# olivier-2018/scene_3Dreconstruction_MVSNet

Hardware: AMD Instinct MI355X
Metric: depth maps/sec at N=5 views, 640x512, D=192; achieved HBM GB/s (higher is better)
Workload: dtype f32 (conv0, conv2-4, conv9, conv11: 3xbf16 split operands on the bf16 matrix cores, fp32 accumulate)

## Files before the change

scene_3dreconstruction_mvsnet_amd/csrc/conv11_prob.hip:

```cpp
#include <cstdlib>

#include "mvs_internal.h"
#include "storage.h"
#include "mfma16_ops.h"

namespace mvs {

namespace cp {
constexpr int BY = 4, BX = 2;
constexpr int IY = 2 * BY, IX = 8 * BX;
constexpr int OY = 2 * IY, OX = 2 * IX;
constexpr int PY = OY - 2, PX = OX - 2;

constexpr int XP = 36;
constexpr int HS = XP * 4, RS = 2 * HS, PS = (OY + 2) * RS;
constexpr int C_FLOATS = 2 * PS;

constexpr int WSLOTS = 69;
__host__ __device__ constexpr int win_slot(int rho, int c) {
    return c < 8 ? 8 * rho + c : rho == 0 ? 52 : rho == 1 ? 48 : rho == 2 ? 56 : rho == 3 ? 60 : rho == 4 ? 68 : 64;
}
}

namespace cpv {
using namespace cp;
constexpr int RPI = 76;
constexpr int WIN = 2 * 3 * RPI;
constexpr int NPC = 2 * 27 * 2;
}

template <int DT>
__global__ __launch_bounds__(512, 4) void conv11_prob_priv_kernel(
    const void* __restrict__ x, const float* __restrict__ bp, const float* __restrict__ bias,
    const void* __restrict__ skip, const float* __restrict__ pw, const float* __restrict__ pbias,
    float* __restrict__ cost, int Di, int Hi, int Wi, int ZC, int nbx, int nby) {
    using namespace cpv;
    __shared__ __attribute__((aligned(16))) float ct[C_FLOATS];
    __shared__ __attribute__((aligned(16))) float win[8 * WIN];
    __shared__ __attribute__((aligned(16))) float bpan[2 * 9 * 64 * 4];

    const int tid = threadIdx.x, lane = tid & 63, wave = tid >> 6;
    int b = xcd_block();
    const int bx = b % nbx; b /= nbx;
    const int by = b % nby;
    const int bz = b / nby;
    const int ix0 = bx * (IX - 1), iy0 = by * (IY - 1);
    const int za = bz * ZC, zb = min(za + ZC, Di);
    const int Do = 2 * Di, Ho = 2 * Hi, Wo = 2 * Wi;
    const size_t Vin = (size_t)Di * Hi * Wi, HWi = (size_t)Hi * Wi, HWo = (size_t)Ho * Wo;
    const int i_first = za > 0 ? za - 1 : 0, i_last = zb < Di ? zb : Di - 1;

    const int tx = wave & 1, ty = wave >> 1;
    float* my = win + wave * WIN;
    int prel[2], ploff[2];
    unsigned pin = 0, phz = 0;
#pragma unroll
    for (int j = 0; j < 2; ++j) {
        const int p = lane + 64 * j;
        const int half = p & 1, v = p >> 1, hz = v / 27, vv = v % 27, hr = vv / 9, hc = vv % 9;
        const int gy = iy0 + 2 * ty + hr, gx = ix0 + 8 * tx + hc;
        const bool ok = p < NPC && gy < Hi && gx < Wi;
        prel[j] = ok ? (int)((((size_t)hz * Hi + gy) * Wi + gx) * 8 + half * 4) : 0;
        pin |= ok ? (1u << j) : 0u;
        phz |= (hz & 1) ? (1u << j) : 0u;
        ploff[j] = p < NPC ? (hz * 3 + hr) * RPI + hc * 8 + half * 4 : -1;
    }
    f32x4 pre[2];
    bool pre_z1 = true;
    auto load_a = [&](int i, int c) {
        pre_z1 = i + 1 < Di;
        const size_t base = ((size_t)c * Vin + (size_t)i * HWi) * 8;
#pragma unroll
        for (int j = 0; j < 2; ++j) {
            const bool ok = ((pin >> j) & 1u) && (pre_z1 || !((phz >> j) & 1u));
            pre[j] = St<DT>::load4(x, ok ? base + prel[j] : (size_t)0);
        }
    };
    auto store_a = [&]() {
#pragma unroll
        for (int j = 0; j < 2; ++j) {
            const bool ok = ((pin >> j) & 1u) && (pre_z1 || !((phz >> j) & 1u));
            if (ploff[j] >= 0) *reinterpret_cast<f32x4*>(my + ploff[j]) = ok ? pre[j] : (f32x4){0.f, 0.f, 0.f, 0.f};
        }
    };
    const int r = lane & 15, g = lane >> 4;
    const int abase = (r >> 3) * RPI + ((r & 7) + (g >> 1)) * 8 + (g & 1) * 4;
    const int px = r >> 3, co = r & 7;
    const float bv = bias[co];
    const int sbase0 = (2 * (2 * ty + (g >> 1)) + 1) * RS + (co >> 2) * HS + (2 * (8 * tx + 4 * (g & 1)) + px + 1) * 4 + (co & 3);
    int srel[4], sl[4];
    unsigned sok = 0;
#pragma unroll
    for (int j = 0; j < 4; ++j) {
        const int xx = lane & 15, half = (lane >> 4) & 1, rr = 2 * (j & 1) + (lane >> 5), pz = j >> 1;
        const int oy = 4 * ty + rr, ox = 16 * tx + xx;
        const int gy = 2 * iy0 + oy, gx = 2 * ix0 + ox;
        const bool ok = gy < Ho && gx < Wo;
        srel[j] = ok ? (int)((((size_t)pz * Ho + gy) * Wo + gx) * 8 + half * 4) : 0;
        sok |= ok ? (1u << j) : 0u;
        sl[j] = pz * PS + (oy + 1) * RS + half * HS + (ox + 1) * 4;
    }
    f32x4 sk[4];
    auto load_skip = [&](int i, bool de, bool dodd) {
        const size_t base = (size_t)(2 * i) * HWo * 8;
#pragma unroll
        for (int j = 0; j < 4; ++j) {
            const bool ok = ((sok >> j) & 1u) && ((j >> 1) ? dodd : de);
            sk[j] = St<DT>::load4(skip, ok ? base + srel[j] : (size_t)0);
        }
    };
    const f32x4* bsrc = reinterpret_cast<const f32x4*>(bpan) + lane;
    f32x4 acc[4];
    auto fetch = [&](int c, int ks, f32x4& a, f32x4& bq) {
        const DeconvStep st = deconv_step(ks);
        a = *reinterpret_cast<const f32x4*>(my + (st.dz * 3 + st.dy) * RPI + abase);
        bq = bsrc[(c * 9 + ks) * 64];
    };
    auto mfma_step = [&](int ks, const f32x4& a, const f32x4& bq) {
        const int cls = deconv_step(ks).cls;
        acc[cls] = __builtin_amdgcn_mfma_f32_16x16x4f32(a.x, bq.x, acc[cls], 0, 0, 0);
        acc[cls] = __builtin_amdgcn_mfma_f32_16x16x4f32(a.y, bq.y, acc[cls], 0, 0, 0);
        acc[cls] = __builtin_amdgcn_mfma_f32_16x16x4f32(a.z, bq.z, acc[cls], 0, 0, 0);
        acc[cls] = __builtin_amdgcn_mfma_f32_16x16x4f32(a.w, bq.w, acc[cls], 0, 0, 0);
    };
    auto mfma_chunk = [&](int c, bool de, bool dodd) {
        if (de && dodd) {
            f32x4 a[2], bq[2];
            fetch(c, 0, a[0], bq[0]);
#pragma unroll
            for (int ks = 0; ks < 9; ++ks) {
                if (ks + 1 < 9) fetch(c, ks + 1, a[(ks + 1) & 1], bq[(ks + 1) & 1]);
                mfma_step(ks, a[ks & 1], bq[ks & 1]);
            }
        } else {
#pragma unroll
            for (int ks = 0; ks < 9; ++ks) {
                if (deconv_step(ks).cls < 2 ? !de : !dodd) continue;
                f32x4 a, bq;
                fetch(c, ks, a, bq);
                mfma_step(ks, a, bq);
            }
        }
    };

    const int lx = tid & 31, ly = tid >> 5;
    const int gyo = 2 * iy0 + ly, gxo = 2 * ix0 + lx;
    const bool pvalid = gyo < Ho && gxo < Wo && (ly >= 1 || iy0 == 0) && (ly <= OY - 2 || gyo == Ho - 1) &&
                        (lx >= 1 || ix0 == 0) && (lx <= OX - 2 || gxo == Wo - 1);
    const size_t pout = (size_t)gyo * Wo + gxo;
    const int cbase = ly * RS + lx * 4;
    auto stencil = [&](int plane, f32x2& k2, f32x2& k1, f32x2& k0) {
        const float* base = ct + plane * PS + cbase;
#pragma unroll 1
        for (int kx = 0; kx < 3; ++kx) {
            f32x4 v[3][2];
#pragma unroll
            for (int rr = 0; rr < 3; ++rr)
#pragma unroll
                for (int hf = 0; hf < 2; ++hf)
                    v[rr][hf] = *reinterpret_cast<const f32x4*>(base + rr * RS + hf * HS + kx * 4);
#pragma unroll
            for (int ky = 0; ky < 3; ++ky) {
                const float* w2 = pw + ((2 * 3 + ky) * 3 + kx) * 8;
                const float* w1 = pw + ((1 * 3 + ky) * 3 + kx) * 8;
                const float* w0 = pw + ((0 * 3 + ky) * 3 + kx) * 8;
#pragma unroll
                for (int c2 = 0; c2 < 4; ++c2) {
                    const f32x4 q = v[ky][c2 >> 1];
                    const f32x2 d = (c2 & 1) ? (f32x2){q.z, q.w} : (f32x2){q.x, q.y};
                    k2 = __builtin_elementwise_fma(d, (f32x2){w2[2 * c2], w2[2 * c2 + 1]}, k2);
                    k1 = __builtin_elementwise_fma(d, (f32x2){w1[2 * c2], w1[2 * c2 + 1]}, k1);
                    k0 = __builtin_elementwise_fma(d, (f32x2){w0[2 * c2], w0[2 * c2 + 1]}, k0);
                }
            }
        }
    };
    const __amdgpu_buffer_rsrc_t crs = __builtin_amdgcn_make_buffer_rsrc(cost, (short)0, (int)((size_t)Do * HWo * 4), 0x00020000);
    auto emit = [&](int oz, const f32x2& sv, bool live) {
        const unsigned off = (pvalid && live) ? (unsigned)(((size_t)oz * HWo + pout) * 4) : 0xFFFFFFFCu;
        __builtin_amdgcn_raw_buffer_store_b32(__builtin_bit_cast(unsigned, sv.x + sv.y), crs, (int)off, 0, 0);
    };

    const float pb = pbias[0];
    const f32x2 fresh = {pb, 0.0f};
    f32x2 A = fresh, B = fresh, C = fresh;

    for (int k = tid; k < C_FLOATS / 4; k += 512) reinterpret_cast<f32x4*>(ct)[k] = (f32x4){0.f, 0.f, 0.f, 0.f};
    for (int k = tid; k < 2 * 9 * 64; k += 512) reinterpret_cast<f32x4*>(bpan)[k] = reinterpret_cast<const f32x4*>(bp)[k];
    load_a(i_first, 0);
    __builtin_amdgcn_sched_barrier(0);
    load_skip(i_first, i_first >= za, i_first < zb);
    __syncthreads();

#pragma unroll 1
    for (int i = i_first; i <= i_last; ++i) {
        const bool de = i >= za, dodd = i < zb;
        store_a();
        __builtin_amdgcn_wave_barrier();
        __builtin_amdgcn_sched_barrier(0);
        load_a(i, 1);
        __builtin_amdgcn_sched_barrier(0);
#pragma unroll
        for (int c = 0; c < 4; ++c) acc[c] = (f32x4){0.f, 0.f, 0.f, 0.f};
        mfma_chunk(0, de, dodd);
        __builtin_amdgcn_wave_barrier();
        __builtin_amdgcn_sched_barrier(0);
        store_a();
        __builtin_amdgcn_wave_barrier();
        __builtin_amdgcn_sched_barrier(0);
        load_a(min(i + 1, i_last), 0);
        __builtin_amdgcn_sched_barrier(0);
        mfma_chunk(1, de, dodd);
#pragma unroll
        for (int c = 0; c < 4; ++c) {
            if (c < 2 ? !de : !dodd) continue;
            float* dst = ct + (c >> 1) * PS + (c & 1) * RS + sbase0;
#pragma unroll
            for (int e = 0; e < 4; ++e) dst[8 * e] = relu(acc[c][e] + bv);
        }
        __builtin_amdgcn_wave_barrier();
#pragma unroll
        for (int pz = 0; pz < 2; ++pz) {
            if (pz ? !dodd : !de) continue;
            f32x4 t[2];
#pragma unroll
            for (int j = 0; j < 2; ++j) t[j] = *reinterpret_cast<const f32x4*>(ct + sl[2 * pz + j]);
#pragma unroll
            for (int j = 0; j < 2; ++j)
                *reinterpret_cast<f32x4*>(ct + sl[2 * pz + j]) =
                    ((sok >> (2 * pz + j)) & 1u) ? t[j] + sk[2 * pz + j] : (f32x4){0.f, 0.f, 0.f, 0.f};
        }
        load_skip(min(i + 1, i_last), true, i + 1 < zb);
        __syncthreads();
        if (de) stencil(0, A, B, C);
        emit(max(2 * i - 1, 0), A, de && i > za);
        A = fresh;
        if (dodd) stencil(1, B, C, A);
        emit(2 * i, B, dodd && de);
        const f32x2 t = A;
        A = C;
        B = t;
        C = fresh;
        __syncthreads();
    }
    emit(Do - 1, A, zb == Di);
}

namespace cpv16 {
using namespace cp;
constexpr int WIN = WSLOTS * 8;
constexpr int NPC = 2 * 27;
}

template <int DT>
__global__ __launch_bounds__(512, 4) void conv11_prob16_kernel(
    const void* __restrict__ x, const unsigned short* __restrict__ bp, const float* __restrict__ bias,
    const void* __restrict__ skip, const float* __restrict__ pw, const float* __restrict__ pbias,
    float* __restrict__ cost, int Di, int Hi, int Wi, int ZC, int nbx, int nby) {
    using namespace cpv16;
    static_assert(DT == MVS_F16 || DT == MVS_BF16, "16-bit storage");
    const unsigned short* xs = static_cast<const unsigned short*>(x);
    const unsigned short* sks = static_cast<const unsigned short*>(skip);
    __shared__ __attribute__((aligned(16))) float ct[C_FLOATS];
    __shared__ __attribute__((aligned(16))) unsigned short win[8 * 2 * WIN];

    const int tid = threadIdx.x, lane = tid & 63, wave = tid >> 6;
    int b = xcd_block();
    const int bx = b % nbx; b /= nbx;
    const int by = b % nby;
    const int bz = b / nby;
    const int ix0 = bx * (IX - 1), iy0 = by * (IY - 1);
    const int za = bz * ZC, zb = min(za + ZC, Di);
    const int Do = 2 * Di, Ho = 2 * Hi, Wo = 2 * Wi;
    const size_t Vin = (size_t)Di * Hi * Wi, HWi = (size_t)Hi * Wi, HWo = (size_t)Ho * Wo;
    const int i_first = za > 0 ? za - 1 : 0, i_last = zb < Di ? zb : Di - 1;

    const int tx = wave & 1, ty = wave >> 1;
    unsigned short* my = win + wave * 2 * WIN;
    const int pv = lane < NPC ? lane : NPC - 1;
    const int phz = pv / 27, pvv = pv % 27, phr = pvv / 9, phc = pvv % 9;
    const int pgy = iy0 + 2 * ty + phr, pgx = ix0 + 8 * tx + phc;
    const bool pin = lane < NPC && pgy < Hi && pgx < Wi;
    const size_t prel = pin ? (((size_t)phz * Hi + pgy) * Wi + pgx) * 8 : 0;
    const int ploff = win_slot(phz * 3 + phr, phc) * 8;
    u32x4 pre[2];
    bool pre_z1 = true;
    auto load_a = [&](int i) {
        pre_z1 = i + 1 < Di;
        const bool ok = pin && (pre_z1 || phz == 0);
#pragma unroll
        for (int c = 0; c < 2; ++c)
            pre[c] = *reinterpret_cast<const u32x4*>(xs + (ok ? ((size_t)c * Vin + (size_t)i * HWi) * 8 + prel : (size_t)0));
    };
    auto store_a = [&]() {
        const bool ok = pin && (pre_z1 || phz == 0);
        if (lane < NPC) {
#pragma unroll
            for (int c = 0; c < 2; ++c)
                *reinterpret_cast<u32x4*>(my + c * WIN + ploff) = ok ? pre[c] : (u32x4){0u, 0u, 0u, 0u};
        }
    };
    const int r = lane & 15, g = lane >> 4;
    int koff[5];
#pragma unroll
    for (int ks = 0; ks < 5; ++ks) {
        const Deconv16Tap t0 = deconv16_tap(ks, 0), t1 = deconv16_tap(ks, 1);
        koff[ks] = win_slot(((g >> 1) ? (t1.dz * 3 + t1.dy) : (t0.dz * 3 + t0.dy)) + (r >> 3), (r & 7) + (g & 1)) * 8;
    }
    const int px = r >> 3, co = r & 7;
    const float bv = bias[co];
    const int sbase0 = (2 * (2 * ty + (g >> 1)) + 1) * RS + (co >> 2) * HS + (2 * (8 * tx + 4 * (g & 1)) + px + 1) * 4 + (co & 3);
    const int sxx = lane & 15, srr = lane >> 4;
    const int soy = 4 * ty + srr, sox = 16 * tx + sxx;
    const bool sok = 2 * iy0 + soy < Ho && 2 * ix0 + sox < Wo;
    const size_t srel = sok ? ((size_t)(2 * iy0 + soy) * Wo + 2 * ix0 + sox) * 8 : 0;
    const int sl = (soy + 1) * RS + (sox + 1) * 4;
    u32x4 sk[2];
    auto load_skip = [&](int i, bool de, bool dodd) {
#pragma unroll
        for (int j = 0; j < 2; ++j) {
            const bool ok = sok && (j ? dodd : de);
            sk[j] = *reinterpret_cast<const u32x4*>(sks + (ok ? (size_t)(2 * i + j) * HWo * 8 + srel : (size_t)0));
        }
    };
    u32x4 breg[2][5];
#pragma unroll
    for (int c = 0; c < 2; ++c)
#pragma unroll
        for (int ks = 0; ks < 5; ++ks) breg[c][ks] = reinterpret_cast<const u32x4*>(bp)[(c * 5 + ks) * 64 + lane];
    f32x4 acc[4];
    auto mfma_all = [&]() {
#pragma unroll
        for (int c = 0; c < 2; ++c)
#pragma unroll
            for (int ks = 0; ks < 5; ++ks) {
                constexpr int dummy = 0;
                (void)dummy;
                const int cls = deconv16_tap(ks, 0).cls;
                const u32x4 a = *reinterpret_cast<const u32x4*>(my + c * WIN + koff[ks]);
                acc[cls] = mfma16<DT>(a, breg[c][ks], acc[cls]);
            }
    };

    const int lx = tid & 31, ly = tid >> 5;
    const int gyo = 2 * iy0 + ly, gxo = 2 * ix0 + lx;
    const bool pvalid = gyo < Ho && gxo < Wo && (ly >= 1 || iy0 == 0) && (ly <= OY - 2 || gyo == Ho - 1) &&
                        (lx >= 1 || ix0 == 0) && (lx <= OX - 2 || gxo == Wo - 1);
    const size_t pout = (size_t)gyo * Wo + gxo;
    const int cbase = ly * RS + lx * 4;
    auto stencil = [&](int plane, f32x2& k2, f32x2& k1, f32x2& k0) {
        const float* base = ct + plane * PS + cbase;
#pragma unroll 1
        for (int kx = 0; kx < 3; ++kx) {
            f32x4 v[3][2];
#pragma unroll
            for (int rr = 0; rr < 3; ++rr)
#pragma unroll
                for (int hf = 0; hf < 2; ++hf)
                    v[rr][hf] = *reinterpret_cast<const f32x4*>(base + rr * RS + hf * HS + kx * 4);
#pragma unroll
            for (int ky = 0; ky < 3; ++ky) {
                const float* w2 = pw + ((2 * 3 + ky) * 3 + kx) * 8;
                const float* w1 = pw + ((1 * 3 + ky) * 3 + kx) * 8;
                const float* w0 = pw + ((0 * 3 + ky) * 3 + kx) * 8;
#pragma unroll
                for (int c2 = 0; c2 < 4; ++c2) {
                    const f32x4 q = v[ky][c2 >> 1];
                    const f32x2 d = (c2 & 1) ? (f32x2){q.z, q.w} : (f32x2){q.x, q.y};
                    k2 = __builtin_elementwise_fma(d, (f32x2){w2[2 * c2], w2[2 * c2 + 1]}, k2);
                    k1 = __builtin_elementwise_fma(d, (f32x2){w1[2 * c2], w1[2 * c2 + 1]}, k1);
                    k0 = __builtin_elementwise_fma(d, (f32x2){w0[2 * c2], w0[2 * c2 + 1]}, k0);
                }
            }
        }
    };
    const __amdgpu_buffer_rsrc_t crs = __builtin_amdgcn_make_buffer_rsrc(cost, (short)0, (int)((size_t)Do * HWo * 4), 0x00020000);
    auto emit = [&](int oz, const f32x2& sv, bool live) {
        const unsigned off = (pvalid && live) ? (unsigned)(((size_t)oz * HWo + pout) * 4) : 0xFFFFFFFCu;
        __builtin_amdgcn_raw_buffer_store_b32(__builtin_bit_cast(unsigned, sv.x + sv.y), crs, (int)off, 0, 0);
    };

    const float pb = pbias[0];
    const f32x2 fresh = {pb, 0.0f};
    f32x2 A = fresh, B = fresh, C = fresh;

    for (int k = tid; k < C_FLOATS / 4; k += 512) reinterpret_cast<f32x4*>(ct)[k] = (f32x4){0.f, 0.f, 0.f, 0.f};
    load_a(i_first);
    __builtin_amdgcn_sched_barrier(0);
    load_skip(i_first, i_first >= za, i_first < zb);
    __syncthreads();

#pragma unroll 1
    for (int i = i_first; i <= i_last; ++i) {
        const bool de = i >= za, dodd = i < zb;
        store_a();
        __builtin_amdgcn_wave_barrier();
        __builtin_amdgcn_sched_barrier(0);
        load_a(min(i + 1, i_last));
        __builtin_amdgcn_sched_barrier(0);
#pragma unroll
        for (int c = 0; c < 4; ++c) acc[c] = (f32x4){0.f, 0.f, 0.f, 0.f};
        mfma_all();
#pragma unroll
        for (int c = 0; c < 4; ++c) {
            if (c < 2 ? !de : !dodd) continue;
            float* dst = ct + (c >> 1) * PS + (c & 1) * RS + sbase0;
#pragma unroll
            for (int e = 0; e < 4; ++e) dst[8 * e] = relu(acc[c][e] + bv);
        }
        __builtin_amdgcn_wave_barrier();
#pragma unroll
        for (int pz = 0; pz < 2; ++pz) {
            if (pz ? !dodd : !de) continue;
            float sv[8];
            unpack8<DT>(sk[pz], sv);
            float* d = ct + pz * PS + sl;
            const f32x4 t0 = *reinterpret_cast<const f32x4*>(d), t1 = *reinterpret_cast<const f32x4*>(d + HS);
            const f32x4 z4 = (f32x4){0.f, 0.f, 0.f, 0.f};
            *reinterpret_cast<f32x4*>(d) = sok ? t0 + (f32x4){sv[0], sv[1], sv[2], sv[3]} : z4;
            *reinterpret_cast<f32x4*>(d + HS) = sok ? t1 + (f32x4){sv[4], sv[5], sv[6], sv[7]} : z4;
        }
        load_skip(min(i + 1, i_last), true, i + 1 < zb);
        __syncthreads();
        if (de) stencil(0, A, B, C);
        emit(max(2 * i - 1, 0), A, de && i > za);
        A = fresh;
        if (dodd) stencil(1, B, C, A);
        emit(2 * i, B, dodd && de);
        const f32x2 t = A;
        A = C;
        B = t;
        C = fresh;
        __syncthreads();
    }
    emit(Do - 1, A, zb == Di);
}

namespace cpvs {
using namespace cp;
constexpr int WIN = WSLOTS * 8;
constexpr int NPC = 2 * 27;
constexpr int PAN = 2 * 5 * 64 * 8;
}

__global__ __launch_bounds__(512, 4) void conv11_prob_split_kernel(
    const float* __restrict__ x, const unsigned short* __restrict__ bp, const float* __restrict__ bias,
    const float* __restrict__ skip, const float* __restrict__ pw, const float* __restrict__ pbias,
    float* __restrict__ cost, int Di, int Hi, int Wi, int ZC, int nbx, int nby) {
    using namespace cpvs;
    __shared__ __attribute__((aligned(16))) float ct[PS];
    __shared__ __attribute__((aligned(16))) unsigned short win[8 * 3 * WIN];
    __shared__ __attribute__((aligned(16))) unsigned short bpan[3 * PAN];

    const int tid = threadIdx.x, lane = tid & 63, wave = tid >> 6;
    int b = xcd_block();
    const int bx = b % nbx; b /= nbx;
    const int by = b % nby;
    const int bz = b / nby;
    const int ix0 = bx * (IX - 1), iy0 = by * (IY - 1);
    const int za = bz * ZC, zb = min(za + ZC, Di);
    const int Do = 2 * Di, Ho = 2 * Hi, Wo = 2 * Wi;
    const size_t Vin = (size_t)Di * Hi * Wi, HWi = (size_t)Hi * Wi, HWo = (size_t)Ho * Wo;
    const int i_first = za > 0 ? za - 1 : 0, i_last = zb < Di ? zb : Di - 1;

    const int tx = wave & 1, ty = wave >> 1;
    unsigned short* my = win + wave * 3 * WIN;
    const int pv = lane < NPC ? lane : NPC - 1;
    const int phz = pv / 27, pvv = pv % 27, phr = pvv / 9, phc = pvv % 9;
    const int pgy = iy0 + 2 * ty + phr, pgx = ix0 + 8 * tx + phc;
    const bool pin = pgy < Hi && pgx < Wi;
    const size_t prel = pin ? (((size_t)phz * Hi + pgy) * Wi + pgx) * 8 : 0;
    const int ploff = win_slot(phz * 3 + phr, phc) * 8;
    f32x4 pre[2];
    bool pre_z1 = true;
    auto load_a = [&](int i, int c) {
        pre_z1 = i + 1 < Di;
        const bool ok = pin && (pre_z1 || phz == 0);
        const float* src = x + (ok ? ((size_t)c * Vin + (size_t)i * HWi) * 8 + prel : (size_t)0);
        pre[0] = *reinterpret_cast<const f32x4*>(src);
        pre[1] = *reinterpret_cast<const f32x4*>(src + 4);
    };
    auto store_a = [&]() {
        const bool ok = pin && (pre_z1 || phz == 0);
        const f32x4 z4 = (f32x4){0.f, 0.f, 0.f, 0.f};
        u32x4 p1, p2, p3;
        gs_split8(ok ? pre[0] : z4, ok ? pre[1] : z4, p1, p2, p3);
        *reinterpret_cast<u32x4*>(my + ploff) = p1;
        *reinterpret_cast<u32x4*>(my + WIN + ploff) = p2;
        *reinterpret_cast<u32x4*>(my + 2 * WIN + ploff) = p3;
    };
    const int r = lane & 15, g = lane >> 4;
    int koff[5];
#pragma unroll
    for (int ks = 0; ks < 5; ++ks) {
        const Deconv16Tap t0 = deconv16_tap(ks, 0), t1 = deconv16_tap(ks, 1);
        koff[ks] = win_slot(((g >> 1) ? (t1.dz * 3 + t1.dy) : (t0.dz * 3 + t0.dy)) + (r >> 3), (r & 7) + (g & 1)) * 8;
    }
    const int px = r >> 3, co = r & 7;
    const float bv = bias[co];
    const int sbase0 = (2 * (2 * ty + (g >> 1)) + 1) * RS + (co >> 2) * HS + (2 * (8 * tx + 4 * (g & 1)) + px + 1) * 4 + (co & 3);
    const int srow = 2 * (iy0 + 2 * ty + (g >> 1)), scol = 2 * (ix0 + 8 * tx + 4 * (g & 1)) + px;
    const unsigned sbase = (unsigned)((((size_t)srow * Wo + scol) * 8 + co) * 4);
    const bool vy0 = srow < Ho, vy1 = srow + 1 < Ho;
    bool vx[4];
#pragma unroll
    for (int e = 0; e < 4; ++e) vx[e] = scol + 2 * e < Wo;
    const __amdgpu_buffer_rsrc_t srs =
        __builtin_amdgcn_make_buffer_rsrc(const_cast<float*>(skip), (short)0, (int)((size_t)Do * HWo * 32), 0x00020000);
    float sk[4][4];
    auto load_skip = [&](int i) {
#pragma unroll
        for (int c = 0; c < 4; ++c) {
            const unsigned so = (unsigned)((((size_t)(2 * i + (c >> 1)) * Ho + (c & 1)) * Wo) * 32);
#pragma unroll
            for (int e = 0; e < 4; ++e)
                sk[c][e] = __builtin_bit_cast(float, __builtin_amdgcn_raw_buffer_load_b32(srs, (int)(sbase + 64 * e), (int)so, 0));
        }
    };
    const u32x4* bsrc = reinterpret_cast<const u32x4*>(bpan) + lane;
    f32x4 acc[4];
    auto mfma_chunk = [&](int c) {
#pragma unroll
        for (int ks = 0; ks < 5; ++ks) {
            const int cls = deconv16_tap(ks, 0).cls;
            const int kq = koff[ks];
            const int bq = c * 5 + ks;
            const u32x4 a1 = *reinterpret_cast<const u32x4*>(my + kq);
            const u32x4 a2 = *reinterpret_cast<const u32x4*>(my + WIN + kq);
            const u32x4 a3 = *reinterpret_cast<const u32x4*>(my + 2 * WIN + kq);
            const u32x4 b1 = bsrc[(0 * 10 + bq) * 64];
            const u32x4 b2 = bsrc[(1 * 10 + bq) * 64];
            const u32x4 b3 = bsrc[(2 * 10 + bq) * 64];
            acc[cls] = mfma16<MVS_BF16>(a3, b1, acc[cls]);
            acc[cls] = mfma16<MVS_BF16>(a1, b3, acc[cls]);
            acc[cls] = mfma16<MVS_BF16>(a2, b2, acc[cls]);
            acc[cls] = mfma16<MVS_BF16>(a2, b1, acc[cls]);
            acc[cls] = mfma16<MVS_BF16>(a1, b2, acc[cls]);
            acc[cls] = mfma16<MVS_BF16>(a1, b1, acc[cls]);
        }
    };
    auto scatter = [&](int pz, const f32x4& s0, const f32x4& s1) {
#pragma unroll
        for (int c = 0; c < 2; ++c) {
            float* dst = ct + c * RS + sbase0;
#pragma unroll
            for (int e = 0; e < 4; ++e) {
                const float v = relu((c ? s1 : s0)[e]) + sk[2 * pz + c][e];
                dst[8 * e] = ((c ? vy1 : vy0) && vx[e]) ? v : 0.0f;
            }
        }
    };

    const int lx = tid & 31, ly = tid >> 5;
    const int gyo = 2 * iy0 + ly, gxo = 2 * ix0 + lx;
    const bool pvalid = gyo < Ho && gxo < Wo && (ly >= 1 || iy0 == 0) && (ly <= OY - 2 || gyo == Ho - 1) &&
                        (lx >= 1 || ix0 == 0) && (lx <= OX - 2 || gxo == Wo - 1);
    const size_t pout = (size_t)gyo * Wo + gxo;
    const int cbase = ly * RS + lx * 4;
    auto stencil = [&](f32x2& k2, f32x2& k1, f32x2& k0) {
        const float* base = ct + cbase;
#pragma unroll 1
        for (int kx = 0; kx < 3; ++kx) {
            f32x4 v[3][2];
#pragma unroll
            for (int rr = 0; rr < 3; ++rr)
#pragma unroll
                for (int hf = 0; hf < 2; ++hf)
                    v[rr][hf] = *reinterpret_cast<const f32x4*>(base + rr * RS + hf * HS + kx * 4);
#pragma unroll
            for (int ky = 0; ky < 3; ++ky) {
                const float* w2 = pw + ((2 * 3 + ky) * 3 + kx) * 8;
                const float* w1 = pw + ((1 * 3 + ky) * 3 + kx) * 8;
                const float* w0 = pw + ((0 * 3 + ky) * 3 + kx) * 8;
#pragma unroll
                for (int c2 = 0; c2 < 4; ++c2) {
                    const f32x4 q = v[ky][c2 >> 1];
                    const f32x2 d = (c2 & 1) ? (f32x2){q.z, q.w} : (f32x2){q.x, q.y};
                    k2 = __builtin_elementwise_fma(d, (f32x2){w2[2 * c2], w2[2 * c2 + 1]}, k2);
                    k1 = __builtin_elementwise_fma(d, (f32x2){w1[2 * c2], w1[2 * c2 + 1]}, k1);
                    k0 = __builtin_elementwise_fma(d, (f32x2){w0[2 * c2], w0[2 * c2 + 1]}, k0);
                }
            }
        }
    };
    const __amdgpu_buffer_rsrc_t crs = __builtin_amdgcn_make_buffer_rsrc(cost, (short)0, (int)((size_t)Do * HWo * 4), 0x00020000);
    auto emit = [&](int oz, const f32x2& sv, bool live) {
        const unsigned off = (pvalid && live) ? (unsigned)(((size_t)oz * HWo + pout) * 4) : 0xFFFFFFFCu;
        __builtin_amdgcn_raw_buffer_store_b32(__builtin_bit_cast(unsigned, sv.x + sv.y), crs, (int)off, 0, 0);
    };

    const float pb = pbias[0];
    const f32x2 fresh = {pb, 0.0f};
    f32x2 A = fresh, B = fresh, C = fresh;

    for (int k = tid; k < PS / 4; k += 512) reinterpret_cast<f32x4*>(ct)[k] = (f32x4){0.f, 0.f, 0.f, 0.f};
    for (int k = tid; k < 3 * PAN / 8; k += 512) reinterpret_cast<u32x4*>(bpan)[k] = reinterpret_cast<const u32x4*>(bp)[k];
    load_a(i_first, 0);
    __builtin_amdgcn_sched_barrier(0);
    load_skip(i_first);
    __syncthreads();

    auto stage = [&](int i_next, int c_next) {
        store_a();
        __builtin_amdgcn_wave_barrier();
        __builtin_amdgcn_sched_barrier(0);
        load_a(i_next, c_next);
        __builtin_amdgcn_sched_barrier(0);
    };
#pragma unroll 1
    for (int i = i_first; i <= i_last; ++i) {
        const bool de = i >= za, dodd = i < zb;
        stage(i, 1);
#pragma unroll
        for (int c = 0; c < 4; ++c) acc[c] = (f32x4){bv, bv, bv, bv};
        mfma_chunk(0);
        __builtin_amdgcn_wave_barrier();
        __builtin_amdgcn_sched_barrier(0);
        stage(min(i + 1, i_last), 0);
        mfma_chunk(1);
        if (de) scatter(0, acc[0], acc[1]);
        __syncthreads();
        if (de) stencil(A, B, C);
        emit(max(2 * i - 1, 0), A, de && i > za);
        A = fresh;
        __syncthreads();
        if (dodd) scatter(1, acc[2], acc[3]);
        load_skip(min(i + 1, i_last));
        __syncthreads();
        if (dodd) stencil(B, C, A);
        emit(2 * i, B, dodd && de);
        const f32x2 t = A;
        A = C;
        B = t;
        C = fresh;
        __syncthreads();
    }
    emit(Do - 1, A, zb == Di);
}

bool conv11_prob_enabled(int dtype) {
    return options().fuse_prob && (dtype == MVS_F32 || mfma16_enabled());
}

int launch_conv11_prob(const void* x, const void* skip, float* cost, const float* blob, int Di, int Hi, int Wi,
                       int dtype, hipStream_t s) {
    using namespace cp;
    if (dtype != MVS_F32 && dtype != MVS_F16 && dtype != MVS_BF16)
        return fail(MVS_ERR_BAD_DTYPE, "conv11_prob: unknown dtype %d", dtype);
    if ((size_t)Di * Hi * Wi * 64 >= ((size_t)1 << 31))
        return fail(MVS_ERR_BAD_SHAPE, "conv11_prob: plane exceeds 31-bit offsets");
    const BlobLayout L = blob_layout();
    const int Ho = 2 * Hi, Wo = 2 * Wi;
    const int nbx = (Wo - 2 + PX - 1) / PX > 0 ? (Wo - 2 + PX - 1) / PX : 1;
    const int nby = (Ho - 2 + PY - 1) / PY > 0 ? (Ho - 2 + PY - 1) / PY : 1;
    const int cus = device_cus();
    const int ntile = nbx * nby, slots = 2 * cus;
    int best = 1;
    double best_eff = 0.0;
    for (int nz = 1; nz <= (Di + 3) / 4; ++nz) {
        const int zc = (Di + nz - 1) / nz, nzc_ = (Di + zc - 1) / zc;
        const long nb = (long)ntile * nzc_;
        const double eff = (double)nb / (double)(((nb + slots - 1) / slots) * slots) * zc / (zc + 1.5);
        if (eff > best_eff + 1e-9) { best_eff = eff; best = nz; }
    }
    int ZC = (Di + best - 1) / best;
    if (ZC < 4) ZC = 4;
    if (ZC > Di) ZC = Di;
    const int nzc = (Di + ZC - 1) / ZC;
    const dim3 grid(nbx * nby * nzc);
    if (dtype == MVS_F32 && options().tail_split && (size_t)Di * Hi * Wi * 256 < ((size_t)1 << 32)) {
        conv11_prob_split_kernel<<<grid, 512, 0, s>>>(
            static_cast<const float*>(x), reinterpret_cast<const unsigned short*>(blob + L.s16_off[9]), blob + L.b_off[9],
            static_cast<const float*>(skip), blob + L.w_off[10], blob + L.b_off[10], cost, Di, Hi, Wi, ZC, nbx, nby);
    } else if (dtype == MVS_F32) {
        conv11_prob_priv_kernel<MVS_F32><<<grid, 512, 0, s>>>(x, blob + L.gp_off[9], blob + L.b_off[9], skip,
                                                               blob + L.w_off[10], blob + L.b_off[10], cost, Di, Hi, Wi,
                                                               ZC, nbx, nby);
    } else {
        const unsigned short* bp16 = reinterpret_cast<const unsigned short*>(blob + L.h16_off[dtype == MVS_F16 ? 0 : 1][9]);
        if (dtype == MVS_F16)
            conv11_prob16_kernel<MVS_F16><<<grid, 512, 0, s>>>(x, bp16, blob + L.b_off[9], skip, blob + L.w_off[10],
                                                               blob + L.b_off[10], cost, Di, Hi, Wi, ZC, nbx, nby);
        else
            conv11_prob16_kernel<MVS_BF16><<<grid, 512, 0, s>>>(x, bp16, blob + L.b_off[9], skip, blob + L.w_off[10],
                                                                blob + L.b_off[10], cost, Di, Hi, Wi, ZC, nbx, nby);
    }
    return check_hip(hipGetLastError(), "conv11_prob launch");
}

}
```

Before: 1550.

## Software-pipeline prob stencil weight loads and trim address arithmetic in conv11

Replaces the per-kernel stencil lambda with a shared prob_plane routine. It double-buffers the 3x8 weight taps per (kx,ky) group and interleaves the next group's weight and LDS row loads with the current FMAs, using explicit waitcnt and sched barriers. Output and input offsets move from 64-bit to 32-bit arithmetic, with pvalid folded into the precomputed byte offset. In the split kernel, invalid-row scatters are redirected to a spare LDS row instead of being masked. The aim is to hide scalar/LDS load latency in the stencil and cut address VALU work, at the cost of more registers, rigid scheduling, and a 32-bit offset overflow risk on large volumes.

New measurement: 1557 (median of 2 runs). No clear change (+0.4%).

```diff
diff --git a/scene_3dreconstruction_mvsnet_amd/csrc/conv11_prob.hip b/scene_3dreconstruction_mvsnet_amd/csrc/conv11_prob.hip
--- a/scene_3dreconstruction_mvsnet_amd/csrc/conv11_prob.hip
+++ b/scene_3dreconstruction_mvsnet_amd/csrc/conv11_prob.hip
@@ -19,6 +19,63 @@
 constexpr int WSLOTS = 69;
 __host__ __device__ constexpr int win_slot(int rho, int c) {
     return c < 8 ? 8 * rho + c : rho == 0 ? 52 : rho == 1 ? 48 : rho == 2 ? 56 : rho == 3 ? 60 : rho == 4 ? 68 : 64;
+}
+
+constexpr int LGKM0 = 0xC07F;
+__device__ __forceinline__ const float* prob_pw_odd(const float* pw) { return __builtin_align_down(pw, 4); }
+
+struct ProbW { float t[3][8]; };
+__device__ __forceinline__ void prob_w_request(ProbW& w, const float* __restrict__ pw, const float* __restrict__ pwo,
+                                               int g, int kz) {
+    const int kx = g / 3, ky = g % 3, m = (kz * 3 + ky) * 3 + kx;
+    const float* src = ((m & 1) ? pwo : pw) + m * 8;
+#pragma unroll
+    for (int c = 0; c < 8; ++c) w.t[kz][c] = src[c];
+}
+
+__device__ __forceinline__ void prob_plane(const float* base, const float* __restrict__ pw, f32x2& k2, f32x2& k1,
+                                           f32x2& k0) {
+    const float* pwo = prob_pw_odd(pw);
+    f32x4 v[3][2];
+    auto row = [&](int kx, int rr) {
+#pragma unroll
+        for (int hf = 0; hf < 2; ++hf) v[rr][hf] = *reinterpret_cast<const f32x4*>(base + rr * RS + hf * HS + kx * 4);
+    };
+    auto taps = [&](const float (&t)[8], int ky, f32x2& k) {
+#pragma unroll
+        for (int c2 = 0; c2 < 4; ++c2) {
+            const f32x4 q = v[ky][c2 >> 1];
+            const f32x2 d = (c2 & 1) ? (f32x2){q.z, q.w} : (f32x2){q.x, q.y};
+            k = __builtin_elementwise_fma(d, (f32x2){t[2 * c2], t[2 * c2 + 1]}, k);
+        }
+    };
+    ProbW set[2];
+#pragma unroll
+    for (int kz = 2; kz >= 0; --kz) prob_w_request(set[0], pw, pwo, 0, kz);
+    row(0, 0);
+    row(0, 1);
+#pragma unroll
+    for (int g = 0; g < 9; ++g) {
+        const int kx = g / 3, ky = g % 3;
+        const ProbW& cur = set[g & 1];
+        ProbW& nxt = set[(g + 1) & 1];
+        __builtin_amdgcn_s_waitcnt(LGKM0);
+        __builtin_amdgcn_sched_barrier(0);
+        if (g + 1 < 9) {
+            prob_w_request(nxt, pw, pwo, g + 1, 2);
+            prob_w_request(nxt, pw, pwo, g + 1, 1);
+        }
+        if (ky == 0) row(kx, 2);
+        else if (kx + 1 < 3) row(kx + 1, ky - 1);
+        __builtin_amdgcn_sched_barrier(0);
+        taps(cur.t[2], ky, k2);
+        __builtin_amdgcn_sched_barrier(0);
+        if (g + 1 < 9) prob_w_request(nxt, pw, pwo, g + 1, 0);
+        __builtin_amdgcn_sched_barrier(0);
+        taps(cur.t[1], ky, k1);
+        taps(cur.t[0], ky, k0);
+        __builtin_amdgcn_sched_barrier(0);
+    }
 }
 }
 
@@ -147,37 +204,11 @@
     const int gyo = 2 * iy0 + ly, gxo = 2 * ix0 + lx;
     const bool pvalid = gyo < Ho && gxo < Wo && (ly >= 1 || iy0 == 0) && (ly <= OY - 2 || gyo == Ho - 1) &&
                         (lx >= 1 || ix0 == 0) && (lx <= OX - 2 || gxo == Wo - 1);
-    const size_t pout = (size_t)gyo * Wo + gxo;
+    const unsigned pout = pvalid ? (unsigned)(gyo * Wo + gxo) * 4u : 0x80000000u;
     const int cbase = ly * RS + lx * 4;
-    auto stencil = [&](int plane, f32x2& k2, f32x2& k1, f32x2& k0) {
-        const float* base = ct + plane * PS + cbase;
-#pragma unroll 1
-        for (int kx = 0; kx < 3; ++kx) {
-            f32x4 v[3][2];
-#pragma unroll
-            for (int rr = 0; rr < 3; ++rr)
-#pragma unroll
-                for (int hf = 0; hf < 2; ++hf)
-                    v[rr][hf] = *reinterpret_cast<const f32x4*>(base + rr * RS + hf * HS + kx * 4);
-#pragma unroll
-            for (int ky = 0; ky < 3; ++ky) {
-                const float* w2 = pw + ((2 * 3 + ky) * 3 + kx) * 8;
-                const float* w1 = pw + ((1 * 3 + ky) * 3 + kx) * 8;
-                const float* w0 = pw + ((0 * 3 + ky) * 3 + kx) * 8;
-#pragma unroll
-                for (int c2 = 0; c2 < 4; ++c2) {
-                    const f32x4 q = v[ky][c2 >> 1];
-                    const f32x2 d = (c2 & 1) ? (f32x2){q.z, q.w} : (f32x2){q.x, q.y};
-                    k2 = __builtin_elementwise_fma(d, (f32x2){w2[2 * c2], w2[2 * c2 + 1]}, k2);
-                    k1 = __builtin_elementwise_fma(d, (f32x2){w1[2 * c2], w1[2 * c2 + 1]}, k1);
-                    k0 = __builtin_elementwise_fma(d, (f32x2){w0[2 * c2], w0[2 * c2 + 1]}, k0);
-                }
-            }
-        }
-    };
     const __amdgpu_buffer_rsrc_t crs = __builtin_amdgcn_make_buffer_rsrc(cost, (short)0, (int)((size_t)Do * HWo * 4), 0x00020000);
     auto emit = [&](int oz, const f32x2& sv, bool live) {
-        const unsigned off = (pvalid && live) ? (unsigned)(((size_t)oz * HWo + pout) * 4) : 0xFFFFFFFCu;
+        const unsigned off = live ? (unsigned)((size_t)oz * HWo * 4) + pout : 0xFFFFFFFCu;
         __builtin_amdgcn_raw_buffer_store_b32(__builtin_bit_cast(unsigned, sv.x + sv.y), crs, (int)off, 0, 0);
     };
 
@@ -232,10 +263,10 @@
         }
         load_skip(min(i + 1, i_last), true, i + 1 < zb);
         __syncthreads();
-        if (de) stencil(0, A, B, C);
+        if (de) prob_plane(ct + cbase, pw, A, B, C);
         emit(max(2 * i - 1, 0), A, de && i > za);
         A = fresh;
-        if (dodd) stencil(1, B, C, A);
+        if (dodd) prob_plane(ct + PS + cbase, pw, B, C, A);
         emit(2 * i, B, dodd && de);
         const f32x2 t = A;
         A = C;
@@ -346,37 +377,11 @@
     const int gyo = 2 * iy0 + ly, gxo = 2 * ix0 + lx;
     const bool pvalid = gyo < Ho && gxo < Wo && (ly >= 1 || iy0 == 0) && (ly <= OY - 2 || gyo == Ho - 1) &&
                         (lx >= 1 || ix0 == 0) && (lx <= OX - 2 || gxo == Wo - 1);
-    const size_t pout = (size_t)gyo * Wo + gxo;
+    const unsigned pout = pvalid ? (unsigned)(gyo * Wo + gxo) * 4u : 0x80000000u;
     const int cbase = ly * RS + lx * 4;
-    auto stencil = [&](int plane, f32x2& k2, f32x2& k1, f32x2& k0) {
-        const float* base = ct + plane * PS + cbase;
-#pragma unroll 1
-        for (int kx = 0; kx < 3; ++kx) {
-            f32x4 v[3][2];
-#pragma unroll
-            for (int rr = 0; rr < 3; ++rr)
-#pragma unroll
-                for (int hf = 0; hf < 2; ++hf)
-                    v[rr][hf] = *reinterpret_cast<const f32x4*>(base + rr * RS + hf * HS + kx * 4);
-#pragma unroll
-            for (int ky = 0; ky < 3; ++ky) {
-                const float* w2 = pw + ((2 * 3 + ky) * 3 + kx) * 8;
-                const float* w1 = pw + ((1 * 3 + ky) * 3 + kx) * 8;
-                const float* w0 = pw + ((0 * 3 + ky) * 3 + kx) * 8;
-#pragma unroll
-                for (int c2 = 0; c2 < 4; ++c2) {
-                    const f32x4 q = v[ky][c2 >> 1];
-                    const f32x2 d = (c2 & 1) ? (f32x2){q.z, q.w} : (f32x2){q.x, q.y};
-                    k2 = __builtin_elementwise_fma(d, (f32x2){w2[2 * c2], w2[2 * c2 + 1]}, k2);
-                    k1 = __builtin_elementwise_fma(d, (f32x2){w1[2 * c2], w1[2 * c2 + 1]}, k1);
-                    k0 = __builtin_elementwise_fma(d, (f32x2){w0[2 * c2], w0[2 * c2 + 1]}, k0);
-                }
-            }
-        }
-    };
     const __amdgpu_buffer_rsrc_t crs = __builtin_amdgcn_make_buffer_rsrc(cost, (short)0, (int)((size_t)Do * HWo * 4), 0x00020000);
     auto emit = [&](int oz, const f32x2& sv, bool live) {
-        const unsigned off = (pvalid && live) ? (unsigned)(((size_t)oz * HWo + pout) * 4) : 0xFFFFFFFCu;
+        const unsigned off = live ? (unsigned)((size_t)oz * HWo * 4) + pout : 0xFFFFFFFCu;
         __builtin_amdgcn_raw_buffer_store_b32(__builtin_bit_cast(unsigned, sv.x + sv.y), crs, (int)off, 0, 0);
     };
 
@@ -422,10 +427,10 @@
         }
         load_skip(min(i + 1, i_last), true, i + 1 < zb);
         __syncthreads();
-        if (de) stencil(0, A, B, C);
+        if (de) prob_plane(ct + cbase, pw, A, B, C);
         emit(max(2 * i - 1, 0), A, de && i > za);
         A = fresh;
-        if (dodd) stencil(1, B, C, A);
+        if (dodd) prob_plane(ct + PS + cbase, pw, B, C, A);
         emit(2 * i, B, dodd && de);
         const f32x2 t = A;
         A = C;
@@ -448,7 +453,7 @@
     const float* __restrict__ skip, const float* __restrict__ pw, const float* __restrict__ pbias,
     float* __restrict__ cost, int Di, int Hi, int Wi, int ZC, int nbx, int nby) {
     using namespace cpvs;
-    __shared__ __attribute__((aligned(16))) float ct[PS];
+    __shared__ __attribute__((aligned(16))) float ct[PS + RS];
     __shared__ __attribute__((aligned(16))) unsigned short win[8 * 3 * WIN];
     __shared__ __attribute__((aligned(16))) unsigned short bpan[3 * PAN];
 
@@ -460,7 +465,8 @@
     const int ix0 = bx * (IX - 1), iy0 = by * (IY - 1);
     const int za = bz * ZC, zb = min(za + ZC, Di);
     const int Do = 2 * Di, Ho = 2 * Hi, Wo = 2 * Wi;
-    const size_t Vin = (size_t)Di * Hi * Wi, HWi = (size_t)Hi * Wi, HWo = (size_t)Ho * Wo;
+    const size_t HWo = (size_t)Ho * Wo;
+    const unsigned Vin8 = (unsigned)(Di * Hi * Wi) * 8u, HWi8 = (unsigned)(Hi * Wi) * 8u;
     const int i_first = za > 0 ? za - 1 : 0, i_last = zb < Di ? zb : Di - 1;
 
     const int tx = wave & 1, ty = wave >> 1;
@@ -469,14 +475,14 @@
     const int phz = pv / 27, pvv = pv % 27, phr = pvv / 9, phc = pvv % 9;
     const int pgy = iy0 + 2 * ty + phr, pgx = ix0 + 8 * tx + phc;
     const bool pin = pgy < Hi && pgx < Wi;
-    const size_t prel = pin ? (((size_t)phz * Hi + pgy) * Wi + pgx) * 8 : 0;
+    const unsigned prel = pin ? (unsigned)((phz * Hi + pgy) * Wi + pgx) * 8u : 0u;
     const int ploff = win_slot(phz * 3 + phr, phc) * 8;
     f32x4 pre[2];
     bool pre_z1 = true;
     auto load_a = [&](int i, int c) {
         pre_z1 = i + 1 < Di;
         const bool ok = pin && (pre_z1 || phz == 0);
-        const float* src = x + (ok ? ((size_t)c * Vin + (size_t)i * HWi) * 8 + prel : (size_t)0);
+        const float* src = x + (ok ? (unsigned)c * Vin8 + (unsigned)i * HWi8 + prel : 0u);
         pre[0] = *reinterpret_cast<const f32x4*>(src);
         pre[1] = *reinterpret_cast<const f32x4*>(src + 4);
     };
@@ -539,14 +545,15 @@
             acc[cls] = mfma16<MVS_BF16>(a1, b1, acc[cls]);
         }
     };
+    const int srow_off[2] = {vy0 ? sbase0 : sbase0 % RS + PS, vy1 ? sbase0 + RS : sbase0 % RS + PS};
     auto scatter = [&](int pz, const f32x4& s0, const f32x4& s1) {
 #pragma unroll
         for (int c = 0; c < 2; ++c) {
-            float* dst = ct + c * RS + sbase0;
+            float* dst = ct + srow_off[c];
 #pragma unroll
             for (int e = 0; e < 4; ++e) {
                 const float v = relu((c ? s1 : s0)[e]) + sk[2 * pz + c][e];
-                dst[8 * e] = ((c ? vy1 : vy0) && vx[e]) ? v : 0.0f;
+                dst[8 * e] = vx[e] ? v : 0.0f;
             }
         }
     };
@@ -555,37 +562,11 @@
     const int gyo = 2 * iy0 + ly, gxo = 2 * ix0 + lx;
     const bool pvalid = gyo < Ho && gxo < Wo && (ly >= 1 || iy0 == 0) && (ly <= OY - 2 || gyo == Ho - 1) &&
                         (lx >= 1 || ix0 == 0) && (lx <= OX - 2 || gxo == Wo - 1);
-    const size_t pout = (size_t)gyo * Wo + gxo;
+    const unsigned pout = pvalid ? (unsigned)(gyo * Wo + gxo) * 4u : 0x80000000u;
     const int cbase = ly * RS + lx * 4;
-    auto stencil = [&](f32x2& k2, f32x2& k1, f32x2& k0) {
-        const float* base = ct + cbase;
-#pragma unroll 1
-        for (int kx = 0; kx < 3; ++kx) {
-            f32x4 v[3][2];
-#pragma unroll
-            for (int rr = 0; rr < 3; ++rr)
-#pragma unroll
-                for (int hf = 0; hf < 2; ++hf)
-                    v[rr][hf] = *reinterpret_cast<const f32x4*>(base + rr * RS + hf * HS + kx * 4);
-#pragma unroll
-            for (int ky = 0; ky < 3; ++ky) {
-                const float* w2 = pw + ((2 * 3 + ky) * 3 + kx) * 8;
-                const float* w1 = pw + ((1 * 3 + ky) * 3 + kx) * 8;
-                const float* w0 = pw + ((0 * 3 + ky) * 3 + kx) * 8;
-#pragma unroll
-                for (int c2 = 0; c2 < 4; ++c2) {
-                    const f32x4 q = v[ky][c2 >> 1];
-                    const f32x2 d = (c2 & 1) ? (f32x2){q.z, q.w} : (f32x2){q.x, q.y};
-                    k2 = __builtin_elementwise_fma(d, (f32x2){w2[2 * c2], w2[2 * c2 + 1]}, k2);
-                    k1 = __builtin_elementwise_fma(d, (f32x2){w1[2 * c2], w1[2 * c2 + 1]}, k1);
-                    k0 = __builtin_elementwise_fma(d, (f32x2){w0[2 * c2], w0[2 * c2 + 1]}, k0);
-                }
-            }
-        }
-    };
     const __amdgpu_buffer_rsrc_t crs = __builtin_amdgcn_make_buffer_rsrc(cost, (short)0, (int)((size_t)Do * HWo * 4), 0x00020000);
     auto emit = [&](int oz, const f32x2& sv, bool live) {
-        const unsigned off = (pvalid && live) ? (unsigned)(((size_t)oz * HWo + pout) * 4) : 0xFFFFFFFCu;
+        const unsigned off = live ? (unsigned)((size_t)oz * HWo * 4) + pout : 0xFFFFFFFCu;
         __builtin_amdgcn_raw_buffer_store_b32(__builtin_bit_cast(unsigned, sv.x + sv.y), crs, (int)off, 0, 0);
     };
 
@@ -620,14 +601,14 @@
         mfma_chunk(1);
         if (de) scatter(0, acc[0], acc[1]);
         __syncthreads();
-        if (de) stencil(A, B, C);
+        if (de) prob_plane(ct + cbase, pw, A, B, C);
         emit(max(2 * i - 1, 0), A, de && i > za);
         A = fresh;
         __syncthreads();
         if (dodd) scatter(1, acc[2], acc[3]);
         load_skip(min(i + 1, i_last));
         __syncthreads();
-        if (dodd) stencil(B, C, A);
+        if (dodd) prob_plane(ct + cbase, pw, B, C, A);
         emit(2 * i, B, dodd && de);
         const f32x2 t = A;
         A = C;
```
